# alpc91/SGRL

Measured on AMD Instinct MI355X. Metric: env-steps/sec (whole node) + SET-actor fwd us/step, 3d_walker mix @8192 envs/GPU, higher is better.
Workload: dtype f64 (dynamics) / f32 (SET actor, obs); 1 GPU; 3D_Walker++ 8 variants x 1024 envs per GPU (config 3), random U(-1,1) actions, auto-reset, SET actor forward on every step, random-init weights; envs_per_gpu=8192, obs_max_len=287, action_max_len=21, replay_gather=none (single rank)

## Files before the change

### include/sgrl_model.h

```cpp
#ifndef SGRL_MODEL_H
#define SGRL_MODEL_H

#include <stdint.h>

#ifdef __HIPCC__
#define SGRL_HD __host__ __device__ inline
#else
#define SGRL_HD static inline
#endif

#define SGRL_MAGIC 0x5347524C
#define SGRL_MAXDEPTH 8

enum {
  SGRL_H_MAGIC = 0,
  SGRL_H_NBODY,
  SGRL_H_NJNT,
  SGRL_H_NQ,
  SGRL_H_NV,
  SGRL_H_NU,
  SGRL_H_NGEOM,
  SGRL_H_NPAIR,
  SGRL_H_INTEGRATOR,
  SGRL_H_FRAME_SKIP,
  SGRL_H_DONE_RULE,
  SGRL_H_TARGET_V2,
  SGRL_H_RESET_VEL_NORMAL,
  SGRL_H_NHEIGHT_BODIES,
  SGRL_H_HEIGHT_BODY0,
  SGRL_H_HEIGHT_BODY1,
  SGRL_H_MAX_ROWS,
  SGRL_H_PGS_ITERS,
  SGRL_H_SOLVER,
  SGRL_NHDR = 24
};

enum {
  SGRL_F_TIMESTEP = 0,
  SGRL_F_GRAV_X, SGRL_F_GRAV_Y, SGRL_F_GRAV_Z,
  SGRL_F_HEIGHT_LO, SGRL_F_HEIGHT_HI, SGRL_F_ANG_LIMIT,
  SGRL_F_ALIVE_BONUS, SGRL_F_HEADING_WEIGHT, SGRL_F_CTRL_COST,
  SGRL_F_RESET_POS_NOISE, SGRL_F_RESET_VEL_NOISE,
  SGRL_F_PGS_TOL,
  SGRL_F_TOTAL_MASS,
  SGRL_NFHDR = 16
};

enum { SGRL_GEOM_PLANE = 0, SGRL_GEOM_SPHERE = 2, SGRL_GEOM_CAPSULE = 3 };
enum { SGRL_JNT_FREE = 0, SGRL_JNT_HINGE = 3 };

#ifndef SGRL_CONST_AS
#define SGRL_CONST_AS
#endif
#ifndef SGRL_ITAB_AS
#define SGRL_ITAB_AS
#endif
#ifndef SGRL_FTAB_AS
#define SGRL_FTAB_AS
#endif
typedef const SGRL_CONST_AS int32_t* sgrl_hdr_t;
typedef const SGRL_CONST_AS double* sgrl_fhdr_t;
typedef const SGRL_ITAB_AS int32_t* sgrl_itab_t;
typedef const SGRL_FTAB_AS double* sgrl_ftab_t;

typedef struct SgrlModelView {
  sgrl_hdr_t hdr;
// ... 111 lines not shown
```

### sgrl_amd/csrc/engine_kernel.h

```cpp
#pragma once
#include <hip/hip_runtime.h>

#include <stdint.h>

#ifndef SGRL_ITAB_GLOBAL
#define SGRL_ITAB_GLOBAL 0
#endif
#ifndef SGRL_STAGE_FLOATS
#define SGRL_STAGE_FLOATS 0
#endif
#if defined(__HIP_DEVICE_COMPILE__)
#define SGRL_CONST_AS __attribute__((address_space(4)))
#if SGRL_ITAB_GLOBAL
#define SGRL_ITAB_AS __attribute__((address_space(4)))
#else
#define SGRL_ITAB_AS __attribute__((address_space(3)))
#endif
#if SGRL_STAGE_FLOATS
#define SGRL_FTAB_AS __attribute__((address_space(3)))
#else
#define SGRL_FTAB_AS __attribute__((address_space(4)))
#endif
#endif
#include "../../include/sgrl.h"
// ... 9 lines not shown


struct BatchArgs {
  const MorphDev* morphs;
  const int32_t* env_morph;
  const int32_t* block_env;
  const int32_t* block_mate;
  double* rec;
  int32_t* cnt;
  double* scratch;
  int scratch_stride;
  int stride;
  int n_env;
  int obs_max_len, action_max_len;
  uint64_t seed;
  uint32_t env_id_base;
  int max_episode_steps;
};

struct StepOut {
  const float* actions;
  float* obs32;
  double* obs64;
  float* reward;
  double* reward64;
  uint8_t* done;
  float* dist;
  uint8_t* truncated;
  int auto_reset;
};


#ifdef SGRL_PHASE_PROF
__device__ unsigned long long g_phase_prof[16 * 65536];
__device__ __forceinline__ unsigned long long* sgrl_phase_prof_buf() { return g_phase_prof; }
#endif

extern __shared__ double sgrl_lds[];

template <class D>
__device__ __forceinline__ void setup(const BatchArgs& a, int env, SgrlModelView* m, sgrl::Layout* o, double** S, int32_t** I) {
  const int mi = __builtin_amdgcn_readfirstlane(a.env_morph[env]);
  const MorphDev md = a.morphs[mi];
  int32_t hdr[SGRL_NHDR];
#pragma unroll
  for (int k = 0; k < SGRL_NHDR; k++) hdr[k] = __builtin_amdgcn_readfirstlane(md.ib[k]);
  D::apply(hdr);
  int n_int, n_f64;
  sgrl_model_blob_sizes(hdr, &n_int, &n_f64);
  sgrl::make_layout(hdr, o, (D::kFixed && SGRL_ITAB_GLOBAL) ? 0 : n_int, SGRL_STAGE_FLOATS ? n_f64 : 0);
  double* s = sgrl_lds;
  int32_t* ii = reinterpret_cast<int32_t*>(sgrl_lds + o->s_total);
  const int lane = threadIdx.x;
  if (SGRL_STAGE_FLOATS) for (int k = lane; k < n_f64; k += 64) s[o->model_f + k] = md.fb[k];
#if !SGRL_ITAB_GLOBAL
  for (int k = lane; k < n_int; k += 64) ii[o->model_i + k] = md.ib[k];
#endif
  __syncthreads();
#if SGRL_STAGE_FLOATS
  sgrl_ftab_t ftab = (sgrl_ftab_t)(s + o->model_f);
#else
  sgrl_ftab_t ftab = (sgrl_ftab_t)md.fb;
#endif
#if SGRL_ITAB_GLOBAL
  sgrl_model_view_dims(hdr, (sgrl_hdr_t)md.ib, (sgrl_fhdr_t)md.fb, (sgrl_itab_t)md.ib, ftab, m);
#else
  sgrl_model_view_dims(hdr, (sgrl_hdr_t)md.ib, (sgrl_fhdr_t)md.fb, (sgrl_itab_t)(ii + o->model_i), ftab, m);
// ... 86 lines not shown
```

### sgrl_amd/csrc/step_body.h

```cpp
#pragma once

#include <math.h>
#include <stdint.h>

#include "../../include/sgrl_model.h"

#ifdef __HIPCC__
#define SGRL_DEV __device__ __forceinline__
#else
#define SGRL_DEV inline
#endif

namespace sgrl {

constexpr double kMinVal = 1e-15;
constexpr double kMinImp = 0.0001;
constexpr double kMaxImp = 0.9999;
constexpr double kPi = 3.14159265358979323846;
constexpr int kNAMax = 32;
constexpr int kBppMaxIter = 40;
constexpr int kSlabRows = 256;
constexpr int kPivotRows = 64;
constexpr int kPrevRows = 48;
constexpr int kSlabLdy = 47;
SGRL_HD int slab_prev_offset(int maxrows, int ldy) { return kPivotRows * (kPivotRows + 1) / 2 + (maxrows + 1) * ldy + 5 * maxrows + 2 * maxrows; }
SGRL_HD int slab_rows_doubles(int maxrows, int ldy) { return slab_prev_offset(maxrows, ldy) + maxrows + maxrows / 2 + 1 + 8; }
SGRL_HD int slab_doubles(int maxrows, int ldy) { return slab_rows_doubles(maxrows, ldy) + ldy * (ldy + 1) / 2; }
constexpr int kScratchDoublesMax = 2080 + 257 * 47 + 7 * 256 + 256 + 129 + 8 + 47 * 48 / 2;

struct Layout {
  int nb, nj, nq, nv, nu, np, ncon, maxrows, lrows, ld, ldy;
  int prevcap;
  int fstride;
  int qpos, qvel, q0, v0, xv, fq, dvacc, daacc, ctrl, act;
  int xpos, xquat, xmat, xipos, xanchor, xaxis;
  int cinert, crb, cdof, cfrc;
// ... 201 lines not shown
  cross3(a, vel, m); cross3(b, vel, m + 3); cross3(c, vel + 3, m);
  r[0] = a[0]; r[1] = a[1]; r[2] = a[2];
  r[3] = b[0] + c[0]; r[4] = b[1] + c[1]; r[5] = b[2] + c[2];
}
SGRL_DEV void cross_force(double* r, const double* vel, const double* f) {
  double a[3], b[3], c[3];
  cross3(a, vel, f); cross3(b, vel + 3, f + 3); cross3(c, vel, f + 3);
  r[0] = a[0] + b[0]; r[1] = a[1] + b[1]; r[2] = a[2] + b[2];
  r[3] = c[0]; r[4] = c[1]; r[5] = c[2];
}
SGRL_DEV void ld3(double* r, const double* p) { r[0] = p[0]; r[1] = p[1]; r[2] = p[2]; }
SGRL_DEV void ld6(double* r, const double* p) { r[0] = p[0]; r[1] = p[1]; r[2] = p[2]; r[3] = p[3]; r[4] = p[4]; r[5] = p[5]; }
SGRL_DEV int popcount64(uint64_t x) {
#ifdef __HIPCC__
  return __popcll(x);
#else
  return __builtin_popcountll(x);
#endif
}
SGRL_DEV int clz64(uint64_t x) {
#ifdef __HIPCC__
  return __clzll((long long)x);
#else
  return __builtin_clzll(x);
#endif
}
SGRL_DEV int tri(int i) { return i * (i + 1) / 2; }
SGRL_DEV void tri_decode(int p, int* a_out, int* b_out) {
  int a = (int)((sqrtf(8.0f * (float)p + 1.0f) - 1.0f) * 0.5f);
  a += ((a + 1) * (a + 2) / 2 <= p) ? 1 : 0;
  a -= (a * (a + 1) / 2 > p) ? 1 : 0;
  *a_out = a; *b_out = p - a * (a + 1) / 2;
}
SGRL_DEV bool dof_in_mask(sgrl_itab_t mask2, int d) {
  const uint32_t w = (uint32_t)(d < 32 ? mask2[0] : mask2[1]);
  return (w >> (d & 31)) & 1u;
}

SGRL_DEV double rng_uniform01(uint64_t seed, uint32_t env_id, uint32_t episode, uint32_t stream, uint32_t idx) {
  uint32_t c0 = idx >> 2, c1 = episode, c2 = stream, c3 = (uint32_t)(seed >> 32);
  uint32_t k0 = (uint32_t)seed, k1 = env_id;
  for (int r = 0; r < 10; r++) {
    const uint64_t p0 = (uint64_t)0xD2511F53u * c0, p1 = (uint64_t)0xCD9E8D57u * c2;
    const uint32_t n0 = (uint32_t)(p1 >> 32) ^ c1 ^ k0, n1 = (uint32_t)p1;
    const uint32_t n2 = (uint32_t)(p0 >> 32) ^ c3 ^ k1, n3 = (uint32_t)p0;
    c0 = n0; c1 = n1; c2 = n2; c3 = n3;
    k0 += 0x9E3779B9u; k1 += 0xBB67AE85u;
  }
  const uint32_t lane = idx & 3u;
  const uint32_t x = lane == 0 ? c0 : (lane == 1 ? c1 : (lane == 2 ? c2 : c3));
  return ((double)x + 0.5) * (1.0 / 4294967296.0);
}

#ifdef SGRL_PHASE_PROF
#define SGRL_TICK(id) w.tick(id)
#else
#define SGRL_TICK(id)
#endif

template <class W>
struct Engine {
  W& w;
  SgrlModelView m;
  const Layout& o;
  double* S;
  int32_t* I;
// ... 161 lines not shown
            cross3(cr, ax, off);
            c[0] = ax[0]; c[1] = ax[1]; c[2] = ax[2]; c[3] = cr[0]; c[4] = cr[1]; c[5] = cr[2];
          }
        } else {
          double ax[3], off[3], cr[3];
          ld3(ax, S + o.xaxis + 3 * j);
          for (int t = 0; t < 3; t++) off[t] = com[t] - S[o.xanchor + 3 * j + t];
          cross3(cr, ax, off);
          c[0] = ax[0]; c[1] = ax[1]; c[2] = ax[2]; c[3] = cr[0]; c[4] = cr[1]; c[5] = cr[2];
        }
      }
    });
  }

  SGRL_DEV void crba_and_factor() {
    const int nv = o.nv;
    w.lanes(o.nb > nv ? o.nb : nv, [&](int i) {
      if (i >= 1 && i < o.nb) {
        double acc[10];
        for (int k = 0; k < 10; k++) acc[k] = 0;
        const int e = m.body_subend[i];
        for (int c = i; c < e; c++)
          for (int k = 0; k < 10; k++) acc[k] += S[o.cinert + 10 * c + k];
        for (int k = 0; k < 10; k++) S[o.crb + 10 * i + k] = acc[k];
      }
      if (i < nv) for (int k = 0; k <= i; k++) S[o.L + tri(i) + k] = 0;
    });
    w.lanes(nv, [&](int i) {
      double buf[6], ci[10], cd[6];
      const int b = m.dof_body[i];
      for (int k = 0; k < 10; k++) ci[k] = S[o.crb + 10 * b + k];
      ld6(cd, S + o.cdof + 6 * i);
      inert_mul(buf, ci, cd);
      S[o.L + tri(i) + i] = dot6(cd, buf) + m.dof_armature[i];
      for (int j = m.dof_parent[i]; j >= 0; j = m.dof_parent[j]) {
        double cj[6];
        ld6(cj, S + o.cdof + 6 * j);
        S[o.L + tri(i) + j] = dot6(cj, buf);
      }
    });
    if (W::hdr_const(m, SGRL_H_INTEGRATOR) == 0) {
      if (o.mfull_hbm) {
        double* const mh = big_scratch + slab_rows_doubles(o.maxrows, o.ldy);
        const int nt = nv * (nv + 1) / 2;
        w.lanes(64, [&](int l) { for (int k = l; k < nt; k += 64) mh[k] = S[o.L + k]; });
      } else {
        w.lanes(nv, [&](int i) { for (int k = 0; k <= i; k++) S[o.Mfull + tri(i) + k] = S[o.L + tri(i) + k]; });
      }
    }
    SGRL_TICK(2);
    linv = w.chol_inv_packed(nv, S + o.L, kMinVal);
    if (!linv) cholesky(o.L);
    SGRL_TICK(8);
  }

  SGRL_DEV void cholesky(int base) {
    const int nv = o.nv;
    for (int j = 0; j < nv - 1; j++) {
      double pj = S[base + tri(j) + j];
      if (pj < kMinVal) pj = kMinVal;
      const double wj = 1.0 / pj;
      const int sdim = nv - j - 1;
      w.lanes(sdim * (sdim + 1) / 2, [&](int p) {
        int a, b;
        tri_decode(p, &a, &b);
        const int i = j + 1 + a, k = j + 1 + b;
        S[base + tri(i) + k] -= S[base + tri(i) + j] * S[base + tri(k) + j] * wj;
      });
    }
    w.lanes(nv, [&](int j) {
      double pj = S[base + tri(j) + j];
      if (pj < kMinVal) pj = kMinVal;
      S[o.dinv + j] = sqrt(1.0 / pj);
    });
    w.lanes(nv * (nv - 1) / 2, [&](int p) {
      int a, b;
      tri_decode(p, &a, &b);
      S[base + tri(a + 1) + b] *= S[o.dinv + b];
    });
  }

  SGRL_DEV void solve_upper_inplace(int base, int xo) { w.trsv_upper(o.nv, S + base, S + o.dinv, S + xo); }
  SGRL_DEV void solve_lower_inplace(int base, int xo) { w.trsv_lower(o.nv, S + base, S + o.dinv, S + xo); }

  SGRL_DEV void geom_pose(int g, double* pos, double* mat) {
    const int b = m.geom_body[g];
// ... 267 lines not shown
        for (int side = -1; side <= 1; side += 2) {
          const double dist = side * (m.jnt_range[2 * j + (side + 1) / 2] - q);
          if (dist >= m.jnt_margin[j]) continue;
          wanted++;
          if (nrow >= maxrows) continue;
          R.kind[nrow] = side < 0 ? ROW_LIMIT_LO : ROW_LIMIT_HI;
          R.src[nrow] = j; R.sub[nrow] = 0;
          nrow++;
        }
      }
      for (int s = 0; s < o.ncon; s++) {
        if (!I[o.con_valid + s]) continue;
        const int p = s >> 1, dim = m.pair_condim[p];
        const int nr = (dim == 1) ? 1 : 2 * (dim - 1);
        wanted += nr;
        if (nrow + nr > maxrows) continue;
        for (int k = 0; k < nr; k++) {
          R.kind[nrow] = dim == 1 ? ROW_CON1 : ROW_PYR;
          R.src[nrow] = s; R.sub[nrow] = k;
          nrow++;
        }
      }
      I[o.icnt + IC_NROW] = nrow; I[o.icnt + IC_NROW_WANTED] = wanted;
      if (wanted > nrow) I[o.icnt + IC_OVERFLOW] += 1;
    });
  }

  template <bool BIG>
  SGRL_DEV void build_rows_and_halfsolve(const Rows& R) {
    const int nv = o.nv, ldy = o.ldy;
    const int nrow = I[o.icnt + IC_NROW];
    w.lanes(nrow + 1, [&](int r) {
      double* Yr = R.Y + r * ldy;
      if (r == nrow) {
        for (int d = 0; d < nv; d++) Yr[d] = S[o.qfs + d];
        return;
      }
      const int kind = R.kind[r], src = R.src[r], sub = R.sub[r];
      double Rreg, aref;
      if (kind == ROW_LIMIT_LO || kind == ROW_LIMIT_HI) {
        const int j = src, side = kind == ROW_LIMIT_LO ? -1 : 1, dof = m.jnt_dofadr[j];
        for (int d = 0; d < nv; d++) Yr[d] = 0;
        Yr[dof] = -side;
        const double q = S[o.qpos + m.jnt_qposadr[j]];
        const double margin = m.jnt_margin[j];
        const double dist = side * (m.jnt_range[2 * j + (side + 1) / 2] - q);
        double si[5], sr[2], K, B;
        for (int k = 0; k < 5; k++) si[k] = m.jnt_solimp[5 * j + k];
        sr[0] = m.jnt_solref[2 * j]; sr[1] = m.jnt_solref[2 * j + 1];
        const double imp = impedance(si, dist - margin);
        kb(sr, si, &K, &B);
        Rreg = (1 - imp) / imp * m.dof_invweight0[dof];
        if (Rreg < kMinVal) Rreg = kMinVal;
        aref = -B * (-side * S[o.qvel + dof]) - K * imp * (dist - margin);
      } else {
        const int s = src, p = s >> 1;
        const int b1 = m.geom_body[m.pair_g1[p]], b2 = m.geom_body[m.pair_g2[p]];
        const double margin = m.pair_margin[p], dist = S[o.con_dist + s], mu = m.pair_mu[p];
        double off[3], dir[3];
        const double* fr = S + o.con_frame + o.fstride * s;
        for (int k = 0; k < 3; k++) off[k] = S[o.con_pos + 3 * s + k] - S[o.misc + MS_COM + k];
        if (kind == ROW_CON1) {
          for (int k = 0; k < 3; k++) dir[k] = fr[k];
        } else {
          const double sg = (sub & 1) ? -mu : mu;
          double tg[3];
          if (sub >> 1) cross3(tg, fr, fr + 3);
          else ld3(tg, fr + 3);
          for (int k = 0; k < 3; k++) dir[k] = fr[k] + sg * tg[k];
        }
        sgrl_itab_t mk1 = m.body_dofmask + 2 * b1;
        sgrl_itab_t mk2 = m.body_dofmask + 2 * b2;
        double vel = 0;
        for (int d = 0; d < nv; d++) {
          double sgn = 0;
          if (b2 > 0 && dof_in_mask(mk2, d)) sgn += 1.0;
          if (b1 > 0 && dof_in_mask(mk1, d)) sgn -= 1.0;
          double val = 0;
          if (sgn != 0) {
            double cd[6], v[3];
            ld6(cd, S + o.cdof + 6 * d);
            cross3(v, cd, off);
            v[0] += cd[3]; v[1] += cd[4]; v[2] += cd[5];
            val = sgn * dot3(dir, v);
          }
          Yr[d] = val;
          vel += val * S[o.qvel + d];
        }
        double si[5], sr[2], K, B;
        for (int k = 0; k < 5; k++) si[k] = m.pair_solimp[5 * p + k];
        sr[0] = m.pair_solref[2 * p]; sr[1] = m.pair_solref[2 * p + 1];
        const double imp = impedance(si, dist - margin);
        kb(sr, si, &K, &B);
        const double tran = m.body_invweight0[2 * b1] + m.body_invweight0[2 * b2];
        if (kind == ROW_CON1) {
          Rreg = (1 - imp) / imp * tran;
          if (Rreg < kMinVal) Rreg = kMinVal;
        } else {
          double R0 = (1 - imp) / imp * (tran + mu * mu * tran);
          if (R0 < kMinVal) R0 = kMinVal;
          Rreg = 2 * mu * mu * R0;
          if (Rreg < kMinVal) Rreg = kMinVal;
        }
        aref = -B * vel - K * imp * (dist - margin);
      }
      R.eR[r] = Rreg; R.earef[r] = aref;
      const int key = (kind << 16) | (src << 3) | sub;
      double f0 = 0;
      const int pn = I[o.icnt + IC_PREV_N];
      const int pcap = o.prevcap, pl = pn < pcap ? pn : pcap;
      for (int k = 0; k < pl; k++) if (I[o.prev_key + k] == key) f0 = S[o.prev_f + k];
      if (pn > pcap) {
        const double* hf = big_scratch + slab_prev_offset(o.maxrows, o.ldy);
        const int32_t* hk = reinterpret_cast<const int32_t*>(hf + o.maxrows);
        for (int k = pcap; k < pn; k++) if (hk[k] == key) f0 = hf[k];
      }
      R.ef[r] = f0;
    });
    SGRL_TICK(6);
// ... 173 lines not shown
      }
      if (!solved) {
        diag_code |= 1;
        if (BIG && nrow > kPivotRows)
          sweeps = w.pgs_big(nrow, nv, R.Y, ldy, R.eb, R.eR, R.eidg, R.ef, S + o.vpgs, m.hdr[SGRL_H_PGS_ITERS], thresh);
        else
          sweeps = w.pgs(nrow, nv, R.Y, ldy, R.eb, R.eR, R.eidg, R.ef, S + o.vpgs, m.hdr[SGRL_H_PGS_ITERS], thresh);
      }
    }
    SGRL_TICK(7);
    const int prevcap = o.prevcap;
    const int nkeep = (nrow <= prevcap || big_scratch != nullptr) ? nrow : prevcap;
    w.lanes(nkeep > 0 ? nkeep : 1, [&](int r) {
      if (r < nkeep) {
        const int key = (R.kind[r] << 16) | (R.src[r] << 3) | R.sub[r];
        if (r < prevcap) {
          I[o.prev_key + r] = key;
          S[o.prev_f + r] = R.ef[r];
        } else {
          double* hf = big_scratch + slab_prev_offset(o.maxrows, o.ldy);
          hf[r] = R.ef[r];
          reinterpret_cast<int32_t*>(hf + o.maxrows)[r] = key;
        }
      }
      if (r == 0) { I[o.icnt + IC_PREV_N] = nkeep; I[o.icnt + IC_SWEEPS] += sweeps; I[o.icnt + IC_ROWSUM] += diag_code; }
    });
    if (linv) {
      w.lanes(nv, [&](int d) { S[o.vpgs + d] = R.Y[nrow * ldy + d] + (nrow > 0 ? S[o.vpgs + d] : 0.0); });
      w.lanes(nv, [&](int k) {
        double s0 = 0, s1 = 0;
        int i = k;
        for (; i + 1 < nv; i += 2) { s0 += S[o.L + tri(i) + k] * S[o.vpgs + i]; s1 += S[o.L + tri(i + 1) + k] * S[o.vpgs + i + 1]; }
        if (i < nv) s0 += S[o.L + tri(i) + k] * S[o.vpgs + i];
        S[o.qacc + k] = s0 + s1;
      });
    } else {
      w.lanes(nv, [&](int d) { S[o.qacc + d] = R.Y[nrow * ldy + d] + (nrow > 0 ? S[o.vpgs + d] : 0.0); });
      solve_upper_inplace(o.L, o.qacc);
    }
  }

  SGRL_DEV void forward() {
    w.fence_lane();
    fence_view();
    SGRL_TICK(-1);
    kinematics();               SGRL_TICK(0);
    com_pos();                  SGRL_TICK(1);
    crba_and_factor();          SGRL_TICK(2);
    collide();                  SGRL_TICK(3);
    bias_and_smooth_force();    SGRL_TICK(4);
    const int wanted = count_rows();
#ifdef SGRL_FORCE_SLAB_ROWS
    if (big_scratch != nullptr) {
#else
    if (wanted > o.lrows && big_scratch != nullptr) {
#endif
      const Rows R = rows_hbm();
      fill_rows(R, wanted, o.maxrows);           SGRL_TICK(5);
      build_rows_and_halfsolve<true>(R);         SGRL_TICK(10);
      pgs_and_finish<true>(R);                   SGRL_TICK(11);
    } else {
      const Rows R = rows_lds();
      fill_rows(R, wanted, o.lrows);             SGRL_TICK(5);
      build_rows_and_halfsolve<false>(R);        SGRL_TICK(10);
      pgs_and_finish<false>(R);                  SGRL_TICK(11);
    }
  }

  SGRL_DEV void integrate_pos(int dst, int src, int vel, double h) {
    w.lanes(o.nj, [&](int j) {
      const int qa = m.jnt_qposadr[j], d = m.jnt_dofadr[j];
// ... 28 lines not shown
          integrate_pos(o.qpos, o.q0, o.xv, a * h);
          w.lanes(nv, [&](int d) {
            const double v = S[o.v0 + d] + a * h * S[o.fq + d];
            S[o.qvel + d] = v; S[o.xv + d] = v;
            S[o.dvacc + d] += bw * v;
          });
        }
        forward();
        if (!rk4) break;
        if (st == 0) {
          w.lanes(nq > nv ? nq : nv, [&](int i) {
            if (i < nq) S[o.q0 + i] = S[o.qpos + i];
            if (i < nv) {
              S[o.v0 + i] = S[o.qvel + i]; S[o.xv + i] = S[o.qvel + i]; S[o.fq + i] = S[o.qacc + i];
              S[o.dvacc + i] = (1.0 / 6) * S[o.qvel + i]; S[o.daacc + i] = (1.0 / 6) * S[o.qacc + i];
            }
          });
        } else {
          w.lanes(nv, [&](int d) { S[o.fq + d] = S[o.qacc + d]; S[o.daacc + d] += bw * S[o.qacc + d]; });
        }
      }
    }
    if (rk4) {
      integrate_pos(o.qpos, o.q0, o.dvacc, h);
      w.lanes(nv, [&](int d) { S[o.qvel + d] = S[o.v0 + d] + h * S[o.daacc + d]; });
    } else {
      if (o.mfull_hbm) {
        const double* const mh = big_scratch + slab_rows_doubles(o.maxrows, o.ldy);
        const int nt = nv * (nv + 1) / 2;
        w.lanes(64, [&](int l) { for (int k = l; k < nt; k += 64) S[o.Mfull + k] = mh[k]; });
      }
      w.lanes(nv, [&](int i) {
        double s = 0;
        for (int j = 0; j < nv; j++) s += (j <= i ? S[o.Mfull + tri(i) + j] : S[o.Mfull + tri(j) + i]) * S[o.qacc + j];
        S[o.fq + i] = s;
      });
      w.lanes(nv, [&](int i) { S[o.Mfull + tri(i) + i] += h * m.dof_damping[i]; });
      cholesky(o.Mfull);
      solve_lower_inplace(o.Mfull, o.fq);
      solve_upper_inplace(o.Mfull, o.fq);
      w.lanes(nv, [&](int d) { S[o.qvel + d] += h * S[o.fq + d]; });
      integrate_pos(o.qpos, o.qpos, o.qvel, h);
    }
  }

  SGRL_DEV void body_velocities() {
    w.lanes(o.nb, [&](int b) {
      double cv[6] = {0, 0, 0, 0, 0, 0};
      if (b > 0) {
        for (int d = m.body_dofadr[b] + m.body_dofnum[b] - 1; d >= 0; d = m.dof_parent[d]) {
          const double qv = S[o.qvel + d];
          for (int k = 0; k < 6; k++) cv[k] += S[o.cdof + 6 * d + k] * qv;
        }
        double off[3], t[3];
        for (int k = 0; k < 3; k++) off[k] = S[o.xpos + 3 * b + k] - S[o.misc + MS_COM + k];
        cross3(t, cv, off);
        cv[3] += t[0]; cv[4] += t[1]; cv[5] += t[2];
      }
      for (int k = 0; k < 6; k++) S[o.cfrc + 6 * b + k] = cv[k];
    });
  }

  SGRL_DEV double obs_element(int b, int k) const {
    const double R2D = 180.0 / kPi;
    if (k < 3) return S[o.xpos + 3 * b + k] - S[o.xpos + 3 + k];
    if (k < 5) return 0.0;
    if (k == 5) return -9.81;
    if (k < 8) {
      const double dx = S[o.misc + 12] - S[o.xpos + 3], dy = S[o.misc + 13] - S[o.xpos + 4];
      const double dn = sqrt(dx * dx + dy * dy);
      return (k == 6 ? dx : dy) / dn;
    }
    if (k == 8) return 0.0;
    if (k < 12) { const double v = S[o.cfrc + 6 * b + 3 + (k - 9)]; return v < -10 ? -10 : (v > 10 ? 10 : v); }
// ... 224 lines not shown
```

### sgrl_amd/csrc/step_spec.hip

```cpp
#include "engine_kernel.h"

#ifndef SGRL_SPEC_ID
#error "compile with -DSGRL_SPEC_ID=<k> -DSGRL_SPEC_WAVES=<w> -DSGRL_SPEC_FAMILY=DimsFixed<...>,..."
#endif
#define SGRL_CAT2(a, b) a##b
#define SGRL_CAT(a, b) SGRL_CAT2(a, b)

namespace {
using namespace sgrl_engine_dev;

__global__ __launch_bounds__(64) __attribute__((amdgpu_waves_per_eu(SGRL_SPEC_WAVES, SGRL_SPEC_WAVES))) void k_env_step_spec(BatchArgs a, StepOut out) {
  const int env = __builtin_amdgcn_readfirstlane(a.block_env[blockIdx.x]);
  const int mate = __builtin_amdgcn_readfirstlane(a.block_mate[blockIdx.x]);
  const int slot = __builtin_amdgcn_readfirstlane(a.morphs[__builtin_amdgcn_readfirstlane(a.env_morph[env])].slot);
  FamilyRun<0, SGRL_SPEC_FAMILY>::run(slot, env, mate, a, out);
}
}

extern "C" int SGRL_CAT(sgrl_spec_launch_, SGRL_SPEC_ID)(int n_wg, int lds, void* stream, const void* batch_args, const void* step_out) {
  static int lds_limit[64];
  static bool init = false;
  if (!init) { for (int& v : lds_limit) v = 48 * 1024; init = true; }
  int dev = 0;
  (void)hipGetDevice(&dev);
  int& limit = lds_limit[dev >= 0 && dev < 64 ? dev : 0];
  if (lds > limit) {
    const hipError_t e = hipFuncSetAttribute(reinterpret_cast<const void*>(k_env_step_spec), hipFuncAttributeMaxDynamicSharedMemorySize, lds);
    if (e != hipSuccess) return (int)e;
    limit = lds;
  }
  hipLaunchKernelGGL(k_env_step_spec, dim3(n_wg), dim3(64), lds, (hipStream_t)stream, *reinterpret_cast<const BatchArgs*>(batch_args),
                     *reinterpret_cast<const StepOut*>(step_out));
  return (int)hipGetLastError();
}
```

### sgrl_amd/csrc/wave_hip.h

```cpp
#pragma once
#include <hip/hip_runtime.h>

#include "../../include/sgrl_model.h"

namespace sgrl {

template <int CTRL>
__device__ __forceinline__ double dpp_move(double x) {
  int lo = __double2loint(x), hi = __double2hiint(x);
  lo = __builtin_amdgcn_update_dpp(0, lo, CTRL, 0xF, 0xF, false);
  hi = __builtin_amdgcn_update_dpp(0, hi, CTRL, 0xF, 0xF, false);
  return __hiloint2double(hi, lo);
}
__device__ __forceinline__ double read_lane(double x, int l) {
  const int lo = __builtin_amdgcn_readlane(__double2loint(x), l);
  const int hi = __builtin_amdgcn_readlane(__double2hiint(x), l);
  return __hiloint2double(hi, lo);
}
__device__ __forceinline__ double wave_sum(double x) {
  x += dpp_move<0xB1>(x);
  x += dpp_move<0x4E>(x);
  x += dpp_move<0x141>(x);
  x += dpp_move<0x140>(x);
  return (read_lane(x, 0) + read_lane(x, 16)) + (read_lane(x, 32) + read_lane(x, 48));
// ... 21 lines not shown
  static_assert(PAIR == 0 || NV <= 15, "two-environments-per-wavefront instances are built for at most 15 dofs");
  __device__ static __forceinline__ void apply(int32_t* hdr) {
    hdr[SGRL_H_NBODY] = NB; hdr[SGRL_H_NJNT] = NJ; hdr[SGRL_H_NQ] = NQ; hdr[SGRL_H_NV] = NV; hdr[SGRL_H_NU] = NU;
    hdr[SGRL_H_NGEOM] = NG; hdr[SGRL_H_NPAIR] = NP; hdr[SGRL_H_INTEGRATOR] = INTEG; hdr[SGRL_H_FRAME_SKIP] = FSKIP;
    hdr[SGRL_H_MAX_ROWS] = MAXROWS; hdr[SGRL_H_SOLVER] = SOLVER;
  }
  template <class M> __device__ static __forceinline__ int hdr_const(const M& m, int idx) {
    return idx == SGRL_H_INTEGRATOR ? INTEG : (idx == SGRL_H_SOLVER ? SOLVER : (idx == SGRL_H_FRAME_SKIP ? FSKIP : m.hdr[idx]));
  }
};

typedef double sgrl_v4d __attribute__((ext_vector_type(4)));
#ifndef SGRL_AFF_MFMA_MIN
#define SGRL_AFF_MFMA_MIN 8
#endif
#ifndef SGRL_TRMM_MFMA_MIN
#define SGRL_TRMM_MFMA_MIN 9
#endif

template <int NVCAP, class D = DimsAny>
struct HipWaveT {
  static constexpr bool kFixedDims = D::kFixed;
  template <class M> __device__ static __forceinline__ int hdr_const(const M& m, int idx) { return D::hdr_const(m, idx); }
  int lane;
#ifdef SGRL_PHASE_PROF
  long long t_last = 0;
  unsigned long long* prof = nullptr;
  __device__ __forceinline__ void tick(int id) {
    const long long t = __builtin_readcyclecounter();
    if (id >= 0 && prof && lane == 0) prof[id] += (unsigned long long)(t - t_last);
    t_last = __builtin_readcyclecounter();
  }
#endif
  __device__ __forceinline__ HipWaveT() : lane(threadIdx.x & 63) {}
  __device__ __forceinline__ void fence_lane() { asm volatile("" : "+v"(lane)); }
  template <class T> __device__ __forceinline__ T fenced(T v) {
    int t = __builtin_amdgcn_readfirstlane((int)(unsigned)(__UINTPTR_TYPE__)v);
    asm volatile("" : "+s"(t));
    return (T)(__UINTPTR_TYPE__)(unsigned)t;
  }
  template <class F> __device__ __forceinline__ void lanes(int n, F f) {
    for (int i = lane; i < n; i += 64) f(i);
    __syncthreads();
  }
  template <class F> __device__ __forceinline__ void lanes_from(int lo, int hi, F f) {
    for (int i = lo + lane; i < hi; i += 64) f(i);
    __syncthreads();
  }
  template <class F> __device__ __forceinline__ double sum(int n, F f) {
    double p = 0.0;
    for (int i = lane; i < n; i += 64) p += f(i);
    return wave_sum(p);
  }
  __device__ __forceinline__ int pgs(int n_in, int nv_in, const double* Y, int ldy, const double* b, const double* R,
                                      const double* idg, double* f, double* v, int iters_in,
                                      double thresh) {
    const int n = __builtin_amdgcn_readfirstlane(n_in), nv = __builtin_amdgcn_readfirstlane(nv_in);
    const int iters = __builtin_amdgcn_readfirstlane(iters_in);
    const bool rowl = lane < n, dofl = lane < nv;
    double rb = rowl ? b[lane] : 0.0, rR = rowl ? R[lane] : 0.0;
    double ridg = rowl ? idg[lane] : 0.0, rf = rowl ? f[lane] : 0.0;
    const double rdg = rowl ? 1.0 / ridg : 0.0;
    double vv = 0.0;
    for (int r = 0; r < n; r++) {
      const double fr = read_lane(rf, r);
      if (dofl) vv += Y[r * ldy + lane] * fr;
// ... 27 lines not shown
    const int n = __builtin_amdgcn_readfirstlane(n_in), nv = __builtin_amdgcn_readfirstlane(nv_in);
    const int iters = __builtin_amdgcn_readfirstlane(iters_in);
    const bool dofl = lane < nv;
    const int dl = dofl ? lane : 0;
    double vv = 0.0;
    for (int r = 0; r < n; r++) {
      const double fr = f[r];
      const double y = Y[r * ldy + dl];
      if (dofl) vv += y * fr;
    }
    int it = 0;
    for (; it < iters; it++) {
      double change = 0.0;
      double yn = Y[dl], bn = b[0], Rn = R[0], in_ = idg[0], fn_ = f[0];
      for (int r = 0; r < n; r++) {
        const double y = dofl ? yn : 0.0, br = bn, Rr = Rn, ir = in_, fr = fn_;
        if (r + 1 < n) { yn = Y[(r + 1) * ldy + dl]; bn = b[r + 1]; Rn = R[r + 1]; in_ = idg[r + 1]; fn_ = f[r + 1]; }
        const double dot = wave_sum(y * vv);
        const double res = br + Rr * fr + dot;
        double fnew = fr - res * ir;
        fnew = fnew < 0.0 ? 0.0 : fnew;
        const double df = fnew - fr;
        vv += y * df;
        if (lane == 0) f[r] = fnew;
        change = fmax(change, fabs(df) / ir);
      }
      __syncthreads();
      if (change < thresh) { it++; break; }
    }
    if (dofl) v[lane] = vv;
    __syncthreads();
    return it;
  }
  template <int NMAX>
  __device__ __forceinline__ void chol_inv_reg(int n, double* P, double minval) {
    const bool act = lane < n;
    const int li = act ? lane : 0;
    double* rowp = P + li * (li + 1) / 2;
    double a[NMAX + 1];
#pragma unroll
    for (int k = 0; k < NMAX; k++) a[k + 1] = rowp[k < li ? k : li];
    double mydj = 0.0;
#pragma unroll
    for (int j = 0; j < NMAX; j++) {
      if (j < n) {
        const double c = a[j + 1];
        double pj = read_lane(c, j);
        pj = pj < minval ? minval : pj;
        const double dj = rsqrt(pj);
        const double l = c * dj;
        mydj = lane == j ? dj : mydj;
        const double lm = lane > j ? l * dj : 0.0;
        a[j] = lane == j ? 1.0 : 0.0;
#pragma unroll
        for (int c2 = 0; c2 <= j; c2++) a[c2] -= lm * read_lane(a[c2], j);
#pragma unroll
        for (int k = j + 1; k < NMAX; k++) a[k + 1] -= l * read_lane(l, k);
      }
    }
    if (act) {
#pragma unroll
      for (int k = NMAX - 1; k >= 0; k--) rowp[k < li ? k : li] = a[k] * mydj;
    }
    __syncthreads();
  }
  __device__ __forceinline__ bool chol_inv_packed(int n_in, double* P, double minval) {
    const int n = __builtin_amdgcn_readfirstlane(n_in);
    if (NVCAP >= 9 && n <= 9) chol_inv_reg<9>(n, P, minval);
    else if (NVCAP >= 12 && n <= 12) chol_inv_reg<12>(n, P, minval);
    else if (NVCAP >= 15 && n <= 15) chol_inv_reg<15>(n, P, minval);
    else if (NVCAP >= 18 && n <= 18) chol_inv_reg<18>(n, P, minval);
    else if (NVCAP >= 21 && n <= 21) chol_inv_reg<21>(n, P, minval);
    else if (NVCAP >= 24 && n <= 24) chol_inv_reg<24>(n, P, minval);
    else return false;
    return true;
  }
  template <int NMAX>
  __device__ __forceinline__ void trmm_rows_reg(int nrhs, int n, const double* T, double* Y, int ldy) {
    constexpr int NH = (NMAX + 1) / 2;
    const int h = lane & 1;
    for (int r0 = 0; r0 < nrhs; r0 += 32) {
      const int r = r0 + (lane >> 1);
      const bool act = r < nrhs;
      double* y = Y + (act ? r : nrhs - 1) * ldy;
      double jr[NH];
#pragma unroll
      for (int u = 0; u < NH; u++) {
        const int c = 2 * u + h;
        const double v = y[c < n ? c : n - 1];
        jr[u] = c < n ? v : 0.0;
      }
#pragma unroll
      for (int d = (NMAX - 1) | 1; d >= 1; d -= 2) {
        if (d - 1 < n) {
          const double* Td = T + d * (d + 1) / 2 + h;
          const double* Te = T + (d - 1) * d / 2 + h;
          double s0 = 0.0, s1 = 0.0, e0 = 0.0, e1 = 0.0;
#pragma unroll
          for (int u = 0; u < NH; u++) {
            if (2 * u + 1 <= d) {
// ... 251 lines not shown
```

### sgrl_amd/model_pack.py

```python
import numpy as np

from . import mjcf
from .env_spec import env_spec_for

NHDR = 24
NFHDR = 16
(H_MAGIC, H_NBODY, H_NJNT, H_NQ, H_NV, H_NU, H_NGEOM, H_NPAIR, H_INTEGRATOR, H_FRAME_SKIP, H_DONE_RULE,
 H_TARGET_V2, H_RESET_VEL_NORMAL, H_NHEIGHT_BODIES, H_HEIGHT_BODY0, H_HEIGHT_BODY1, H_MAX_ROWS,
 H_PGS_ITERS, H_SOLVER) = range(19)
(F_TIMESTEP, F_GRAV_X, F_GRAV_Y, F_GRAV_Z, F_HEIGHT_LO, F_HEIGHT_HI, F_ANG_LIMIT, F_ALIVE_BONUS,
 F_HEADING_WEIGHT, F_CTRL_COST, F_RESET_POS_NOISE, F_RESET_VEL_NOISE, F_PGS_TOL, F_TOTAL_MASS) = range(14)

DEFAULT_MAX_ROWS = 48
DEFAULT_PGS_ITERS = 300
DEFAULT_PGS_TOL = 1e-10
DEFAULT_SOLVER = 1


MAXDEPTH = 8


def _derived_int_tables(model):
    nb, nv = model.nbody, model.nv
    depth = np.zeros(nb, dtype=np.int32)
    path = np.full((nb, MAXDEPTH), -1, dtype=np.int32)
    subend = np.zeros(nb, dtype=np.int32)
    mask = np.zeros((nb, 2), dtype=np.int32)
    for b in range(1, nb):
        chain = []
        a = b
        while a > 0:
            chain.append(a)
            a = int(model.body_parent[a])
        chain.reverse()
        if len(chain) > MAXDEPTH:
            raise ValueError("kinematic chain deeper than %d" % MAXDEPTH)
        depth[b] = len(chain)
        path[b, :len(chain)] = chain
        bits = 0
        for c in chain:
            for d in range(int(model.body_dofadr[c]), int(model.body_dofadr[c]) + int(model.body_dofnum[c])):
                bits |= 1 << d
        lo, hi = bits & 0xFFFFFFFF, (bits >> 32) & 0xFFFFFFFF
        mask[b] = np.array([lo, hi], dtype=np.uint32).view(np.int32)
    for b in range(nb - 1, 0, -1):
        subend[b] = max(subend[b], b + 1)
        p = int(model.body_parent[b])
        if p > 0:
            subend[p] = max(subend[p], subend[b])
    for b in range(1, nb):
        for c in range(b + 1, nb):
            inside = c < subend[b]
            a = c
            anc = False
            while a > 0:
                if a == b:
                    anc = True
                a = int(model.body_parent[a])
            if inside != anc:
                raise ValueError("bodies are not in pre-order")
    if nv > 64:
        raise ValueError("nv > 64 unsupported")
    dof_act = np.full(nv, -1, dtype=np.int32)
    for u in range(model.nu):
        dof_act[int(model.act_dof[u])] = u
    return [depth, path.ravel(), subend, mask.ravel(), dof_act]


def worst_case_rows(model):
    rows = int(np.sum(np.asarray(model.jnt_limited) != 0))
    for k in range(model.npair):
        g2 = int(model.pair_g2[k])
        ncon = 2 if (int(model.geom_type[int(model.pair_g1[k])]) == mjcf.GEOM_PLANE and int(model.geom_type[g2]) == mjcf.GEOM_CAPSULE) else 1
        dim = int(model.pair_condim[k])
        rows += ncon * (1 if dim == 1 else 2 * (dim - 1))
    return rows


def pack_model(model, spec=None, env_name=None, max_rows=DEFAULT_MAX_ROWS, pgs_iters=DEFAULT_PGS_ITERS,
               pgs_tol=DEFAULT_PGS_TOL, solver=DEFAULT_SOLVER):
    if spec is None:
        spec = env_spec_for(env_name or model.name)
    hdr = np.zeros(NHDR, dtype=np.int32)
    hdr[H_MAGIC] = mjcf.MAGIC
    hdr[H_NBODY], hdr[H_NJNT], hdr[H_NQ], hdr[H_NV] = model.nbody, model.njnt, model.nq, model.nv
    hdr[H_NU], hdr[H_NGEOM], hdr[H_NPAIR] = model.nu, model.ngeom, model.npair
    hdr[H_INTEGRATOR] = model.integrator
    hdr[H_FRAME_SKIP] = spec.frame_skip
    hdr[H_DONE_RULE] = spec.done_rule
    hdr[H_TARGET_V2] = 1 if spec.target_v2 else 0
    hdr[H_RESET_VEL_NORMAL] = 1 if spec.reset_vel_normal else 0
    hb = [model.body_names.index(n) for n in spec.height_bodies if n in model.body_names]
    hdr[H_NHEIGHT_BODIES] = len(hb)
    for i, b in enumerate(hb[:2]):
        hdr[H_HEIGHT_BODY0 + i] = b
    hdr[H_MAX_ROWS] = min(int(max_rows), max(1, worst_case_rows(model)))
    hdr[H_PGS_ITERS] = pgs_iters
    hdr[H_SOLVER] = solver
    ints = [hdr]
    for k in mjcf.Model.INT_FIELDS:
        ints.append(np.asarray(getattr(model, k), dtype=np.int32).ravel())
    ints.extend(_derived_int_tables(model))
    fh = np.zeros(NFHDR, dtype=np.float64)
    fh[F_TIMESTEP] = model.timestep
    fh[F_GRAV_X:F_GRAV_Z + 1] = model.gravity
    fh[F_HEIGHT_LO], fh[F_HEIGHT_HI], fh[F_ANG_LIMIT] = spec.height_lo, spec.height_hi, spec.ang_limit
    fh[F_ALIVE_BONUS], fh[F_HEADING_WEIGHT], fh[F_CTRL_COST] = spec.alive_bonus, spec.heading_weight, spec.ctrl_cost
    fh[F_RESET_POS_NOISE], fh[F_RESET_VEL_NOISE] = spec.reset_pos_noise, spec.reset_vel_noise
    fh[F_PGS_TOL] = pgs_tol
    fh[F_TOTAL_MASS] = float(np.sum(model.body_mass[1:]))
    fls = [fh]
    for k in mjcf.Model.F64_FIELDS:
        fls.append(np.asarray(getattr(model, k), dtype=np.float64).ravel())
    return np.ascontiguousarray(np.concatenate(ints)), np.ascontiguousarray(np.concatenate(fls))
```

Measured before the change: 1.982 million env-steps/s.

## Reverse DOF ordering in mass matrix and exploit leg tree sparsity in Cholesky inverse

Stores the joint-space mass matrix with dof indices reversed, so the root's free-joint dofs come last and fill-in from the Cholesky factorisation is reduced. The two final leg subtrees are detected at pack time and recorded in new header fields. Specialised register Cholesky-inverse instantiations then skip updates that are structurally zero between independent legs. Constraint rows, solves and implicit integration are remapped to the reversed slots, which risks indexing bugs. Phase-profiling symbol linkage is also adjusted.

Result: no change. 2.000 million env-steps/s (median of 6 runs) (+0.9%).

```diff
diff --git a/include/sgrl_model.h b/include/sgrl_model.h
--- a/include/sgrl_model.h
+++ b/include/sgrl_model.h
@@ -32,6 +32,8 @@
   SGRL_H_MAX_ROWS,
   SGRL_H_PGS_ITERS,
   SGRL_H_SOLVER,
+  SGRL_H_LEG_A,
+  SGRL_H_LEG_B,
   SGRL_NHDR = 24
 };
 
diff --git a/sgrl_amd/csrc/engine_kernel.h b/sgrl_amd/csrc/engine_kernel.h
--- a/sgrl_amd/csrc/engine_kernel.h
+++ b/sgrl_amd/csrc/engine_kernel.h
@@ -65,7 +65,10 @@
 
 
 #ifdef SGRL_PHASE_PROF
-__device__ unsigned long long g_phase_prof[16 * 65536];
+#ifndef SGRL_PHASE_PROF_LINKAGE
+#define SGRL_PHASE_PROF_LINKAGE
+#endif
+SGRL_PHASE_PROF_LINKAGE __device__ unsigned long long g_phase_prof[16 * 65536];
 __device__ __forceinline__ unsigned long long* sgrl_phase_prof_buf() { return g_phase_prof; }
 #endif
 
diff --git a/sgrl_amd/csrc/step_body.h b/sgrl_amd/csrc/step_body.h
--- a/sgrl_amd/csrc/step_body.h
+++ b/sgrl_amd/csrc/step_body.h
@@ -2,6 +2,9 @@
 
 #include <math.h>
 #include <stdint.h>
+
+#include <type_traits>
+#include <utility>
 
 #include "../../include/sgrl_model.h"
 
@@ -269,6 +272,10 @@
   a -= (a * (a + 1) / 2 > p) ? 1 : 0;
   *a_out = a; *b_out = p - a * (a + 1) / 2;
 }
+SGRL_DEV int dof_slot(int nv, int d) { return nv - 1 - d; }
+template <class W, class = void> struct HasTreeLegs : std::false_type {};
+template <class W> struct HasTreeLegs<W, std::void_t<decltype(std::declval<W&>().tree_legs(0, 0))>> : std::true_type {};
+
 SGRL_DEV bool dof_in_mask(sgrl_itab_t mask2, int d) {
   const uint32_t w = (uint32_t)(d < 32 ? mask2[0] : mask2[1]);
   return (w >> (d & 31)) & 1u;
@@ -496,11 +503,12 @@
       for (int k = 0; k < 10; k++) ci[k] = S[o.crb + 10 * b + k];
       ld6(cd, S + o.cdof + 6 * i);
       inert_mul(buf, ci, cd);
-      S[o.L + tri(i) + i] = dot6(cd, buf) + m.dof_armature[i];
+      const int si = dof_slot(nv, i);
+      S[o.L + tri(si) + si] = dot6(cd, buf) + m.dof_armature[i];
       for (int j = m.dof_parent[i]; j >= 0; j = m.dof_parent[j]) {
         double cj[6];
         ld6(cj, S + o.cdof + 6 * j);
-        S[o.L + tri(i) + j] = dot6(cj, buf);
+        S[o.L + tri(dof_slot(nv, j)) + si] = dot6(cj, buf);
       }
     });
     if (W::hdr_const(m, SGRL_H_INTEGRATOR) == 0) {
@@ -513,9 +521,17 @@
       }
     }
     SGRL_TICK(2);
+    tree_legs(true);
     linv = w.chol_inv_packed(nv, S + o.L, kMinVal);
+    tree_legs(false);
     if (!linv) cholesky(o.L);
     SGRL_TICK(8);
+  }
+  SGRL_DEV void tree_legs(bool on) {
+    if constexpr (HasTreeLegs<W>::value) {
+      if (on) w.tree_legs(m.hdr[SGRL_H_LEG_A], m.hdr[SGRL_H_LEG_B]);
+      else w.tree_legs(0, 0);
+    }
   }
 
   SGRL_DEV void cholesky(int base) {
@@ -849,8 +865,9 @@
     const int nrow = I[o.icnt + IC_NROW];
     w.lanes(nrow + 1, [&](int r) {
       double* Yr = R.Y + r * ldy;
+      double* const Ye = Yr + dof_slot(nv, 0);
       if (r == nrow) {
-        for (int d = 0; d < nv; d++) Yr[d] = S[o.qfs + d];
+        for (int d = 0; d < nv; d++) Ye[-d] = S[o.qfs + d];
         return;
       }
       const int kind = R.kind[r], src = R.src[r], sub = R.sub[r];
@@ -858,7 +875,7 @@
       if (kind == ROW_LIMIT_LO || kind == ROW_LIMIT_HI) {
         const int j = src, side = kind == ROW_LIMIT_LO ? -1 : 1, dof = m.jnt_dofadr[j];
         for (int d = 0; d < nv; d++) Yr[d] = 0;
-        Yr[dof] = -side;
+        Yr[dof_slot(nv, dof)] = -side;
         const double q = S[o.qpos + m.jnt_qposadr[j]];
         const double margin = m.jnt_margin[j];
         const double dist = side * (m.jnt_range[2 * j + (side + 1) / 2] - q);
@@ -901,7 +918,7 @@
             v[0] += cd[3]; v[1] += cd[4]; v[2] += cd[5];
             val = sgn * dot3(dir, v);
           }
-          Yr[d] = val;
+          Ye[-d] = val;
           vel += val * S[o.qvel + d];
         }
         double si[5], sr[2], K, B;
@@ -1141,11 +1158,12 @@
         int i = k;
         for (; i + 1 < nv; i += 2) { s0 += S[o.L + tri(i) + k] * S[o.vpgs + i]; s1 += S[o.L + tri(i + 1) + k] * S[o.vpgs + i + 1]; }
         if (i < nv) s0 += S[o.L + tri(i) + k] * S[o.vpgs + i];
-        S[o.qacc + k] = s0 + s1;
+        S[o.qacc + dof_slot(nv, k)] = s0 + s1;
       });
     } else {
-      w.lanes(nv, [&](int d) { S[o.qacc + d] = R.Y[nrow * ldy + d] + (nrow > 0 ? S[o.vpgs + d] : 0.0); });
-      solve_upper_inplace(o.L, o.qacc);
+      w.lanes(nv, [&](int d) { S[o.vpgs + d] = R.Y[nrow * ldy + d] + (nrow > 0 ? S[o.vpgs + d] : 0.0); });
+      solve_upper_inplace(o.L, o.vpgs);
+      w.lanes(nv, [&](int d) { S[o.qacc + d] = S[o.vpgs + dof_slot(nv, d)]; });
     }
   }
 
@@ -1240,14 +1258,14 @@
       }
       w.lanes(nv, [&](int i) {
         double s = 0;
-        for (int j = 0; j < nv; j++) s += (j <= i ? S[o.Mfull + tri(i) + j] : S[o.Mfull + tri(j) + i]) * S[o.qacc + j];
+        for (int j = 0; j < nv; j++) s += (j <= i ? S[o.Mfull + tri(i) + j] : S[o.Mfull + tri(j) + i]) * S[o.qacc + dof_slot(nv, j)];
         S[o.fq + i] = s;
       });
-      w.lanes(nv, [&](int i) { S[o.Mfull + tri(i) + i] += h * m.dof_damping[i]; });
+      w.lanes(nv, [&](int i) { S[o.Mfull + tri(i) + i] += h * m.dof_damping[dof_slot(nv, i)]; });
       cholesky(o.Mfull);
       solve_lower_inplace(o.Mfull, o.fq);
       solve_upper_inplace(o.Mfull, o.fq);
-      w.lanes(nv, [&](int d) { S[o.qvel + d] += h * S[o.fq + d]; });
+      w.lanes(nv, [&](int d) { S[o.qvel + d] += h * S[o.fq + dof_slot(nv, d)]; });
       integrate_pos(o.qpos, o.qpos, o.qvel, h);
     }
   }
diff --git a/sgrl_amd/csrc/step_spec.hip b/sgrl_amd/csrc/step_spec.hip
--- a/sgrl_amd/csrc/step_spec.hip
+++ b/sgrl_amd/csrc/step_spec.hip
@@ -1,3 +1,6 @@
+#ifdef SGRL_PHASE_PROF
+#define SGRL_PHASE_PROF_LINKAGE static
+#endif
 #include "engine_kernel.h"
 
 #ifndef SGRL_SPEC_ID
@@ -33,3 +36,16 @@
                      *reinterpret_cast<const StepOut*>(step_out));
   return (int)hipGetLastError();
 }
+
+#ifdef SGRL_PHASE_PROF
+extern "C" int SGRL_CAT(sgrl_spec_phase_prof_, SGRL_SPEC_ID)(unsigned long long* host, int n_env, int reset) {
+  if (hipDeviceSynchronize() != hipSuccess) return -1;
+  if (n_env < 0 || n_env > 65536) return -4;
+  if (host && hipMemcpyFromSymbol(host, HIP_SYMBOL(sgrl_engine_dev::g_phase_prof), sizeof(unsigned long long) * 16 * (size_t)n_env) != hipSuccess) return -2;
+  if (reset) {
+    static unsigned long long z[16 * 65536];
+    if (hipMemcpyToSymbol(HIP_SYMBOL(sgrl_engine_dev::g_phase_prof), z, sizeof(z)) != hipSuccess) return -3;
+  }
+  return 0;
+}
+#endif
diff --git a/sgrl_amd/csrc/wave_hip.h b/sgrl_amd/csrc/wave_hip.h
--- a/sgrl_amd/csrc/wave_hip.h
+++ b/sgrl_amd/csrc/wave_hip.h
@@ -77,6 +77,10 @@
     t_last = __builtin_readcyclecounter();
   }
 #endif
+  int leg_a = 0, leg_b = 0;
+  __device__ __forceinline__ void tree_legs(int a, int b) {
+    leg_a = __builtin_amdgcn_readfirstlane(a); leg_b = __builtin_amdgcn_readfirstlane(b);
+  }
   __device__ __forceinline__ HipWaveT() : lane(threadIdx.x & 63) {}
   __device__ __forceinline__ void fence_lane() { asm volatile("" : "+v"(lane)); }
   template <class T> __device__ __forceinline__ T fenced(T v) {
@@ -170,8 +174,9 @@
     __syncthreads();
     return it;
   }
-  template <int NMAX>
+  template <int NMAX, int LA = 0, int LB = 0>
   __device__ __forceinline__ void chol_inv_reg(int n, double* P, double minval) {
+    static_assert(LA >= 0 && LB >= 0 && LA + LB <= NMAX, "leg sizes");
     const bool act = lane < n;
     const int li = act ? lane : 0;
     double* rowp = P + li * (li + 1) / 2;
@@ -191,9 +196,11 @@
         const double lm = lane > j ? l * dj : 0.0;
         a[j] = lane == j ? 1.0 : 0.0;
 #pragma unroll
-        for (int c2 = 0; c2 <= j; c2++) a[c2] -= lm * read_lane(a[c2], j);
-#pragma unroll
-        for (int k = j + 1; k < NMAX; k++) a[k + 1] -= l * read_lane(l, k);
+        for (int c2 = 0; c2 <= j; c2++)
+          if (!(LA > 0 && j >= LB && j < LB + LA && c2 < LB)) a[c2] -= lm * read_lane(a[c2], j);
+#pragma unroll
+        for (int k = j + 1; k < NMAX; k++)
+          if (!(LA > 0 && j < LB && k >= LB && k < LB + LA)) a[k + 1] -= l * read_lane(l, k);
       }
     }
     if (act) {
@@ -204,6 +211,12 @@
   }
   __device__ __forceinline__ bool chol_inv_packed(int n_in, double* P, double minval) {
     const int n = __builtin_amdgcn_readfirstlane(n_in);
+    if (D::kFixed && leg_a > 0 && 6 + leg_a + leg_b == n) {
+      if (NVCAP == 18 && n == 18 && leg_a == 6 && leg_b == 6) { chol_inv_reg<18, 6, 6>(n, P, minval); return true; }
+      if (NVCAP == 18 && n == 18 && leg_a == 9 && leg_b == 3) { chol_inv_reg<18, 9, 3>(n, P, minval); return true; }
+      if (NVCAP == 21 && n == 21 && leg_a == 6 && leg_b == 9) { chol_inv_reg<21, 6, 9>(n, P, minval); return true; }
+      if (NVCAP == 24 && n == 24 && leg_a == 9 && leg_b == 9) { chol_inv_reg<24, 9, 9>(n, P, minval); return true; }
+    }
     if (NVCAP >= 9 && n <= 9) chol_inv_reg<9>(n, P, minval);
     else if (NVCAP >= 12 && n <= 12) chol_inv_reg<12>(n, P, minval);
     else if (NVCAP >= 15 && n <= 15) chol_inv_reg<15>(n, P, minval);
diff --git a/sgrl_amd/model_pack.py b/sgrl_amd/model_pack.py
--- a/sgrl_amd/model_pack.py
+++ b/sgrl_amd/model_pack.py
@@ -7,7 +7,7 @@
 NFHDR = 16
 (H_MAGIC, H_NBODY, H_NJNT, H_NQ, H_NV, H_NU, H_NGEOM, H_NPAIR, H_INTEGRATOR, H_FRAME_SKIP, H_DONE_RULE,
  H_TARGET_V2, H_RESET_VEL_NORMAL, H_NHEIGHT_BODIES, H_HEIGHT_BODY0, H_HEIGHT_BODY1, H_MAX_ROWS,
- H_PGS_ITERS, H_SOLVER) = range(19)
+ H_PGS_ITERS, H_SOLVER, H_LEG_A, H_LEG_B) = range(21)
 (F_TIMESTEP, F_GRAV_X, F_GRAV_Y, F_GRAV_Z, F_HEIGHT_LO, F_HEIGHT_HI, F_ANG_LIMIT, F_ALIVE_BONUS,
  F_HEADING_WEIGHT, F_CTRL_COST, F_RESET_POS_NOISE, F_RESET_VEL_NOISE, F_PGS_TOL, F_TOTAL_MASS) = range(14)
 
@@ -67,6 +67,20 @@
     return [depth, path.ravel(), subend, mask.ravel(), dof_act]
 
 
+def tree_legs(dof_parent, nroot):
+    dof_parent = [int(p) for p in dof_parent]
+    nv = len(dof_parent)
+    starts = [d for d in range(nroot, nv) if dof_parent[d] < nroot]
+    if nroot <= 0 or len(starts) < 2:
+        return 0, 0
+    s1, s2 = starts[-2], starts[-1]
+    for d in range(s1, nv):
+        lo = s1 if d < s2 else s2
+        if d not in (s1, s2) and not lo <= dof_parent[d] < d:
+            return 0, 0
+    return s2 - s1, nv - s2
+
+
 def worst_case_rows(model):
     rows = int(np.sum(np.asarray(model.jnt_limited) != 0))
     for k in range(model.npair):
@@ -97,6 +111,7 @@
     hdr[H_MAX_ROWS] = min(int(max_rows), max(1, worst_case_rows(model)))
     hdr[H_PGS_ITERS] = pgs_iters
     hdr[H_SOLVER] = solver
+    hdr[H_LEG_A], hdr[H_LEG_B] = tree_legs(model.dof_parent, int(model.body_dofnum[1]))
     ints = [hdr]
     for k in mjcf.Model.INT_FIELDS:
         ints.append(np.asarray(getattr(model, k), dtype=np.int32).ravel())
```
